# peach-xiao/EMRT

Measured on AMD Instinct MI355X. Metric: training tiles/sec at 256x256, higher is better.
Workload: dtype bf16; 1 GPU; EMRT ResNet50, Potsdam 256x256, 6 classes, batch 8 per GPU, fwd+bwd+SGD step (BASELINE configs[1]), bf16; global_batch=8, parallelism=dp1, hipgraph=True

## Files before the change

emrt_amd/csrc/bn_operand.hpp:

```cpp
#pragma once
#include "common.hpp"

namespace emrt {

#define BN_REPLICAS 8
__device__ __forceinline__ double rep_sum(const double* __restrict__ sums, int C, int idx) {
  double t = 0.0;
#pragma unroll
  for (int r = 0; r < BN_REPLICAS; ++r) t += sums[(long long)r * 2 * C + idx];
  return t;
}

struct BnChan { float mean, invstd; };
__device__ __forceinline__ BnChan bn_chan(const double* __restrict__ sums, const float* __restrict__ run_mean,
                                          const float* __restrict__ run_var, int C, int c, double inv_count, float eps) {
  BnChan o;
  if (sums) {
    const double mu = rep_sum(sums, C, c) * inv_count;
    double var = rep_sum(sums, C, C + c) * inv_count - mu * mu;
    if (var < 0.0) var = 0.0;
    o.mean = (float)mu;
    o.invstd = (float)(1.0 / sqrt(var + (double)eps));
  } else {
    o.mean = run_mean[c];
    o.invstd = rsqrtf(run_var[c] + eps);
  }
  return o;
}

__device__ __forceinline__ void bn_scale_shift(float mean, float invstd, float gamma, float beta, float& scale, float& shift) {
  scale = invstd * gamma;
  shift = fmaf(-mean, scale, beta);
}

struct BnOperand {
  const double* sums;
  double inv_count;
  float eps, momentum;
  float* mean;
  float* invstd;
  float* run_mean;
  float* run_var;
  const float* gamma;
  const float* beta;
  int relu;
};

__device__ __forceinline__ void bn_operand_preamble(const BnOperand& b, int C, float* lds, bool first) {
  for (int ch = threadIdx.x; ch < C; ch += blockDim.x) {
    const BnChan k = bn_chan(b.sums, nullptr, nullptr, C, ch, b.inv_count, b.eps);
    float sc, sh;
    bn_scale_shift(k.mean, k.invstd, b.gamma[ch], b.beta[ch], sc, sh);
    lds[ch] = sc;
    lds[C + ch] = sh;
    if (first) {
      b.mean[ch] = k.mean;
      b.invstd[ch] = k.invstd;
      if (b.run_mean) {
        const double mu = rep_sum(b.sums, C, ch) * b.inv_count;
        double var = rep_sum(b.sums, C, C + ch) * b.inv_count - mu * mu;
        if (var < 0.0) var = 0.0;
        b.run_mean[ch] = b.momentum * b.run_mean[ch] + (1.f - b.momentum) * (float)mu;
        b.run_var[ch] = b.momentum * b.run_var[ch] + (1.f - b.momentum) * (float)var;
      }
    }
  }
  __syncthreads();
}

}
```

emrt_amd/csrc/common.hpp:

```cpp
#pragma once
#include <hip/hip_runtime.h>
#include <stdint.h>
#include <stdio.h>
#include <string.h>
#include "../../include/emrt_hip.h"

#define EMRT_F32 0
#define EMRT_BF16 1
#define EMRT_F16 2

namespace emrt {

extern thread_local char g_err[512];
inline int fail(const char* fn, const char* msg) {
  snprintf(g_err, sizeof(g_err), "%s: %s", fn, msg);
  return -1;
}
inline int check_launch(const char* fn) {
  hipError_t e = hipGetLastError();
  if (e != hipSuccess) {
    snprintf(g_err, sizeof(g_err), "%s: launch failed: %s", fn, hipGetErrorString(e));
    return -2;
  }
  return 0;
}
#define EMRT_REQUIRE(cond, msg) \
  do {                          \
    if (!(cond)) return emrt::fail(__func__, msg); \
  } while (0)

struct Tuning {
  int conv_tile;
  int wgrad_split;
  int thin_cblk;
  int thin_blocks;
  int thin_ch;
  int no_thin_bwd;
  int igemm64_nst;
  int wgrad_nst;
  int pair_max;
  int msda_fwd_global;
  int msda_bwd_global;
  int msda_lds_min_pairs;
  int msda_bwd_dref_lds;
  int msda_band_halo;
  int msda_scatter_qsplit;
  int msda_scatter_cuts;
  int msda_fwd_chunks;
  int msda_fwd_threads;
  int msda_fwd_probe;
  int bn_block_kb;
  int bn_operand_blocks;
  int ln_bwd_rows;
  int ln_bwd_max_blocks;
  int ln_bwd_threads;
  int ln_atomic;
  int gn_group_blocks;
  int gn_stat_rows;
  int gn_bwd_stat_rows;
  int gn_apply_rows;
  int igemm8p_probe;
  int igemm8p_cmajor;
  int igemm8p_min_blocks;
  int wgrad8p_min_steps;
  int wgrad8p_slab;
  int wgrad8p_xcd;
  int wgrad8p_force;
  int no_ksplit128;
  int wgrad_no_overwrite;
  int no_s2_dgrad;
  int wgroup_blocks;
  int wgroup_min_steps;
  int wgroup_max;
  int wgroup8;
  int wgroup8_blocks;
  int wgroup8_min_work;
  int msda_scatter_merge;
  int msda_scatter_mfma;
  int msda_mf_bands;
  int sgd_nt;
  int mha_bwd_split;
  int mha_valu;
  int no_bna;
  int memcpy_kernel;
  int xk;
};
extern Tuning g_tune;

struct Scratch {
  void* ptr; size_t bytes; void* stream;
  unsigned* tick;
  float* xk_part;
};
constexpr size_t SCRATCH_TICK_BYTES = 65536;
constexpr int SCRATCH_TICKS = (int)(SCRATCH_TICK_BYTES / 4);
constexpr size_t SCRATCH_XK_BYTES = 8u << 20;
extern Scratch g_scratch;

struct bf16_t {
  unsigned short v;
};
struct f16_t {
  unsigned short v;
};

__device__ __forceinline__ float to_f32(float x) { return x; }
__device__ __forceinline__ float to_f32(bf16_t x) { return __uint_as_float(((uint32_t)x.v) << 16); }
__device__ __forceinline__ float to_f32(f16_t x) { return (float)__builtin_bit_cast(_Float16, x.v); }
__device__ __forceinline__ float bf16_bits_to_f32(uint32_t lo16) { return __uint_as_float(lo16 << 16); }
__device__ __forceinline__ float f16_bits_to_f32(uint32_t lo16) { return (float)__builtin_bit_cast(_Float16, (unsigned short)lo16); }

template <class T>
__device__ __forceinline__ T from_f32(float f);
template <>
__device__ __forceinline__ float from_f32<float>(float f) {
  return f;
}
template <>
__device__ __forceinline__ bf16_t from_f32<bf16_t>(float f) {
  __bf16 b = (__bf16)f;
  bf16_t r;
  r.v = __builtin_bit_cast(unsigned short, b);
  return r;
}
template <>
__device__ __forceinline__ f16_t from_f32<f16_t>(float f) {
  f16_t r;
  r.v = __builtin_bit_cast(unsigned short, (_Float16)f);
  return r;
}
typedef __attribute__((ext_vector_type(2))) _Float16 emrt_half2_t;
typedef __attribute__((ext_vector_type(2))) float emrt_float2_t;
__device__ __forceinline__ uint32_t pack_f16x2(float lo, float hi) {
  emrt_half2_t h = __builtin_convertvector((emrt_float2_t){lo, hi}, emrt_half2_t);
// ... 252 lines not shown
```

emrt_amd/csrc/elementwise.hip:

```cpp
#include "common.hpp"
#include <stdlib.h>

using namespace emrt;

thread_local char emrt::g_err[512] = {0};

extern "C" const char* emrt_last_error(void) { return emrt::g_err; }
extern "C" int emrt_abi_version(void) { return 9; }

namespace {
struct TuneEntry { const char* name; int emrt::Tuning::*field; int def; };
const TuneEntry kTune[] = {
    {"conv_tile", &emrt::Tuning::conv_tile, 0},         {"wgrad_split", &emrt::Tuning::wgrad_split, 0},
    {"thin_cblk", &emrt::Tuning::thin_cblk, 64},        {"thin_blocks", &emrt::Tuning::thin_blocks, 128},
    {"thin_ch", &emrt::Tuning::thin_ch, 8},             {"no_thin_bwd", &emrt::Tuning::no_thin_bwd, 0},
    {"pair_max", &emrt::Tuning::pair_max, 768},         {"msda_fwd_global", &emrt::Tuning::msda_fwd_global, 0},
    {"bn_block_kb", &emrt::Tuning::bn_block_kb, 8},     {"ln_atomic", &emrt::Tuning::ln_atomic, 1},
    {"msda_fwd_chunks", &emrt::Tuning::msda_fwd_chunks, 0}, {"msda_fwd_threads", &emrt::Tuning::msda_fwd_threads, 1024},
    {"msda_fwd_probe", &emrt::Tuning::msda_fwd_probe, 0}, {"wgrad_nst", &emrt::Tuning::wgrad_nst, 2},
    {"igemm64_nst", &emrt::Tuning::igemm64_nst, 3}, {"msda_bwd_global", &emrt::Tuning::msda_bwd_global, 0},
    {"msda_lds_min_pairs", &emrt::Tuning::msda_lds_min_pairs, 2048}, {"msda_bwd_dref_lds", &emrt::Tuning::msda_bwd_dref_lds, 1},
    {"gn_group_blocks", &emrt::Tuning::gn_group_blocks, 0}, {"gn_stat_rows", &emrt::Tuning::gn_stat_rows, 32},
    {"gn_bwd_stat_rows", &emrt::Tuning::gn_bwd_stat_rows, 32}, {"gn_apply_rows", &emrt::Tuning::gn_apply_rows, 8},
    {"msda_scatter_cuts", &emrt::Tuning::msda_scatter_cuts, 0}, {"msda_scatter_qsplit", &emrt::Tuning::msda_scatter_qsplit, 0}, {"msda_band_halo", &emrt::Tuning::msda_band_halo, 0},
    {"igemm8p_probe", &emrt::Tuning::igemm8p_probe, 0}, {"igemm8p_min_blocks", &emrt::Tuning::igemm8p_min_blocks, 160}, {"igemm8p_cmajor", &emrt::Tuning::igemm8p_cmajor, 0},
    {"wgrad8p_min_steps", &emrt::Tuning::wgrad8p_min_steps, 8}, {"wgrad8p_slab", &emrt::Tuning::wgrad8p_slab, 1}, {"wgrad8p_force", &emrt::Tuning::wgrad8p_force, 0}, {"wgrad8p_xcd", &emrt::Tuning::wgrad8p_xcd, 1},
    {"wgrad_no_overwrite", &emrt::Tuning::wgrad_no_overwrite, 0}, {"no_ksplit128", &emrt::Tuning::no_ksplit128, 0}, {"ln_bwd_rows", &emrt::Tuning::ln_bwd_rows, 0}, {"ln_bwd_max_blocks", &emrt::Tuning::ln_bwd_max_blocks, 0}, {"bn_operand_blocks", &emrt::Tuning::bn_operand_blocks, 0}, {"no_s2_dgrad", &emrt::Tuning::no_s2_dgrad, 0}, {"wgroup_blocks", &emrt::Tuning::wgroup_blocks, 1024}, {"wgroup_min_steps", &emrt::Tuning::wgroup_min_steps, 32}, {"wgroup_max", &emrt::Tuning::wgroup_max, 0},
    {"no_bna", &emrt::Tuning::no_bna, 0}, {"memcpy_kernel", &emrt::Tuning::memcpy_kernel, 0}, {"xk", &emrt::Tuning::xk, 0}, {"mha_valu", &emrt::Tuning::mha_valu, 0}, {"mha_bwd_split", &emrt::Tuning::mha_bwd_split, 1}, {"msda_scatter_merge", &emrt::Tuning::msda_scatter_merge, 0},
    {"wgroup8", &emrt::Tuning::wgroup8, 0}, {"wgroup8_blocks", &emrt::Tuning::wgroup8_blocks, 0}, {"wgroup8_min_work", &emrt::Tuning::wgroup8_min_work, 6000},
    {"msda_scatter_mfma", &emrt::Tuning::msda_scatter_mfma, 1}, {"sgd_nt", &emrt::Tuning::sgd_nt, 1}, {"ln_bwd_threads", &emrt::Tuning::ln_bwd_threads, 512}, {"msda_mf_bands", &emrt::Tuning::msda_mf_bands, 0},
};
emrt::Tuning tuning_from_env() {
  emrt::Tuning t;
  for (const TuneEntry& e : kTune) {
    char env[64] = "EMRT_";
    size_t n = strlen(env);
    for (const char* c = e.name; *c && n + 1 < sizeof(env); ++c) env[n++] = (char)((*c >= 'a' && *c <= 'z') ? *c - 32 : *c);
    env[n] = 0;
    const char* v = (strcmp(e.name, "msda_fwd_probe") == 0 || strcmp(e.name, "igemm8p_probe") == 0) ? nullptr : getenv(env);
    t.*(e.field) = v ? atoi(v) : e.def;
  }
  return t;
}
}
emrt::Tuning emrt::g_tune = tuning_from_env();
emrt::Scratch emrt::g_scratch = {nullptr, 0, nullptr, nullptr, nullptr};

extern "C" int emrt_set_scratch(void* ptr, size_t bytes, void* stream) {
  EMRT_REQUIRE((ptr != nullptr) == (bytes > 0) && ((uintptr_t)ptr) % 256 == 0, "scratch must be 256-byte aligned device memory (or nullptr, 0)");
  if (ptr && ptr == emrt::g_scratch.ptr && emrt::g_scratch.tick && bytes == emrt::g_scratch.bytes + emrt::SCRATCH_TICK_BYTES + emrt::SCRATCH_XK_BYTES) {
    emrt::g_scratch.stream = stream;
    return 0;
  }
  emrt::g_scratch.ptr = ptr;
  emrt::g_scratch.bytes = bytes;
  emrt::g_scratch.stream = stream;
  emrt::g_scratch.tick = nullptr;
  emrt::g_scratch.xk_part = nullptr;
  if (ptr && bytes >= (16u << 20) + emrt::SCRATCH_XK_BYTES + emrt::SCRATCH_TICK_BYTES && bytes % 256 == 0) {
    emrt::g_scratch.bytes = bytes - emrt::SCRATCH_TICK_BYTES - emrt::SCRATCH_XK_BYTES;
    emrt::g_scratch.xk_part = reinterpret_cast<float*>(static_cast<char*>(ptr) + emrt::g_scratch.bytes);
    emrt::g_scratch.tick = reinterpret_cast<unsigned*>(static_cast<char*>(ptr) + emrt::g_scratch.bytes + emrt::SCRATCH_XK_BYTES);
    if (hipMemsetAsync(emrt::g_scratch.tick, 0, emrt::SCRATCH_TICK_BYTES, (hipStream_t)stream) != hipSuccess) {
      emrt::g_scratch.tick = nullptr;
      return emrt::fail("emrt_set_scratch", "cannot zero the arrival counters");
    }
  }
  return 0;
}

extern "C" int emrt_set_tuning(const char* name, int value) {
  EMRT_REQUIRE(name, "null name");
  for (const TuneEntry& e : kTune)
    if (strcmp(e.name, name) == 0) { emrt::g_tune.*(e.field) = value; return 0; }
  return emrt::fail("emrt_set_tuning", "unknown knob");
}
extern "C" int emrt_get_tuning(const char* name, int* value) {
  EMRT_REQUIRE(name && value, "null pointer");
  for (const TuneEntry& e : kTune)
    if (strcmp(e.name, name) == 0) { *value = emrt::g_tune.*(e.field); return 0; }
  return emrt::fail("emrt_get_tuning", "unknown knob");
}

static inline int ew_grid(long long total) {
  long long g = (total + 255) / 256;
  if (g > 8192) g = 8192;
  if (g < 1) g = 1;
  return (int)g;
}

template <class T>
__global__ __launch_bounds__(256) void add_kernel(const T* __restrict__ a, const T* __restrict__ b, T* __restrict__ out, long long n4,
                                                  long long period4) {
  for (long long i = (long long)blockIdx.x * blockDim.x + threadIdx.x; i < n4; i += (long long)gridDim.x * blockDim.x) {
    float x[4], y[4];
    Vec4<T>::load(a + i * 4, x);
    Vec4<T>::load(b + ((n4 | period4) <= 0xffffffffll ? (long long)((unsigned)i % (unsigned)period4) : i % period4) * 4, y);
#pragma unroll
    for (int e = 0; e < 4; ++e) x[e] += y[e];
    Vec4<T>::store(out + i * 4, x);
// ... 381 lines not shown
```

emrt_amd/csrc/norm.hip:

```cpp
#include "common.hpp"
#include "bn_operand.hpp"
#include <stdlib.h>

using namespace emrt;

template <class T, int MODE>
__global__ __launch_bounds__(256) void col_reduce_kernel(const T* __restrict__ x, int ldx, const T* __restrict__ dy, int lddy,
                                                         const T* __restrict__ y, int ldy, const float* __restrict__ mean,
                                                         const float* __restrict__ invstd, long long M, int C, int tx_n,
                                                         float* __restrict__ partial, long long rpb, long long bs,
                                                         double* __restrict__ dsums, float* __restrict__ facc,
                                                         const float* __restrict__ mgamma = nullptr, const float* __restrict__ mbeta = nullptr) {
  __shared__ float red[256 * 8];
  const int ty_n = 256 / tx_n;
  const int tx = threadIdx.x % tx_n, ty = threadIdx.x / tx_n;
  const int c = (blockIdx.y * tx_n + tx) * 4;
  float s0[4] = {0, 0, 0, 0}, s1[4] = {0, 0, 0, 0};
  if (c < C) {
    float mu[4] = {0, 0, 0, 0}, is[4] = {1, 1, 1, 1};
    float msc[MODE == 3 ? 4 : 1], msh[MODE == 3 ? 4 : 1];
    if (MODE == 1 || MODE == 3) {
#pragma unroll
      for (int e = 0; e < 4; ++e) { mu[e] = mean[c + e]; is[e] = invstd[c + e]; }
      if constexpr (MODE == 3) {
// ... 44 lines not shown
  if (ty == 0 && c < C) {
    for (int t = 1; t < ty_n; ++t) {
#pragma unroll
      for (int e = 0; e < 4; ++e) { s0[e] += red[(t * tx_n + tx) * 8 + e]; s1[e] += red[(t * tx_n + tx) * 8 + 4 + e]; }
    }
    if (dsums) {
      double* rep = dsums + (long long)(blockIdx.x & 7) * 2 * C;
#pragma unroll
      for (int e = 0; e < 4; ++e) { atomicAdd(rep + c + e, (double)s0[e]); atomicAdd(rep + C + c + e, (double)s1[e]); }
    } else if (facc) {
#pragma unroll
      for (int e = 0; e < 4; ++e)
        if (c + e < C) atomicAdd(facc + c + e, s0[e]);
    } else {
      float* pp = partial + (long long)blockIdx.x * 2 * C;
#pragma unroll
      for (int e = 0; e < 4; ++e) { pp[c + e] = s0[e]; pp[C + c + e] = s1[e]; }
    }
  }
}

static inline void col_reduce_geometry(long long M, int C, int& tx_n, int& gx, int& gy) {
  int quads = (C + 3) / 4;
  tx_n = 64;
  while (tx_n > 1 && tx_n / 2 >= quads) tx_n /= 2;
  gy = (quads + tx_n - 1) / tx_n;
  int ty_n = 256 / tx_n;
  long long want = (M + (long long)ty_n * 8 - 1) / ((long long)ty_n * 8);
  long long cap = 512 / gy;
  if (cap < 1) cap = 1;
  gx = (int)(want < 1 ? 1 : (want > cap ? cap : want));
}

__global__ __launch_bounds__(256) void bn_sum_partials_kernel(const float* __restrict__ partial, int nblk, int C, float* __restrict__ sums ) {
  __shared__ double red[8][33];
  const int cx = threadIdx.x & 31, py = threadIdx.x >> 5;
  const int c = blockIdx.x * 32 + cx;
  double s = 0.0;
  if (c < 2 * C)
    for (int b = py; b < nblk; b += 8) s += (double)partial[(long long)b * 2 * C + c];
  red[py][cx] = s;
  __syncthreads();
  if (py == 0 && c < 2 * C) {
    double t = 0.0;
#pragma unroll
    for (int k = 0; k < 8; ++k) t += red[k][cx];
    sums[c] = (float)t;
  }
}

__global__ __launch_bounds__(256) void partials_acc_kernel(const float* __restrict__ partial, int nblk, int C, float* __restrict__ dgamma,
                                                          float* __restrict__ dbeta) {
  __shared__ double red[8][33];
  const int cx = threadIdx.x & 31, py = threadIdx.x >> 5;
  const int c = blockIdx.x * 32 + cx;
  double s = 0.0;
  if (c < 2 * C)
    for (int b = py; b < nblk; b += 8) s += (double)partial[(long long)b * 2 * C + c];
  red[py][cx] = s;
  __syncthreads();
  if (py == 0 && c < 2 * C) {
    double t = 0.0;
#pragma unroll
    for (int k = 0; k < 8; ++k) t += red[k][cx];
    if (c < C) { if (dbeta) dbeta[c] += (float)t; }
    else if (dgamma) dgamma[c - C] += (float)t;
  }
}

__global__ void bn_bwd_finalize_kernel(const float* __restrict__ sums, int C, float* __restrict__ dgamma, float* __restrict__ dbeta) {
  const int c = blockIdx.x * blockDim.x + threadIdx.x;
  if (c >= C) return;
  if (dbeta) dbeta[c] += sums[c];
  if (dgamma) dgamma[c] += sums[C + c];
}

template <class T, bool JOIN = false>
__global__ __launch_bounds__(512) void bn_apply_kernel(const T* __restrict__ x, int ldx, const T* __restrict__ res, int ldres,
                                                       T* __restrict__ y, int ldy, const double* __restrict__ sums, double inv_count,
                                                       float eps, float momentum, float* __restrict__ mean_out,
                                                       float* __restrict__ invstd_out, float* __restrict__ run_mean,
                                                       float* __restrict__ run_var, const float* __restrict__ gamma,
                                                       const float* __restrict__ beta, long long M, int C, int relu, int rows_per_pass,
                                                       BnOperand rbn) {
  const int quads = C / 4;
  const int c = (threadIdx.x % quads) * 4;
  const int lane_row = threadIdx.x / quads;
  const long long rstep = (long long)gridDim.x * rows_per_pass;
  long long r = (long long)blockIdx.x * rows_per_pass + lane_row;
  float v[4], w[4];
  if (r < M) {
    Vec4<T>::load(x + r * ldx + c, v);
    if (res) Vec4<T>::load(res + r * ldres + c, w);
  }
  extern __shared__ float bn_lds[];
  if constexpr (JOIN) bn_operand_preamble(rbn, C, bn_lds + 2 * C, blockIdx.x == 0);
  for (int ch = threadIdx.x; ch < C; ch += blockDim.x) {
    const BnChan k = bn_chan(sums, run_mean, run_var, C, ch, inv_count, eps);
    float scale, shift;
    bn_scale_shift(k.mean, k.invstd, gamma[ch], beta[ch], scale, shift);
    bn_lds[ch] = scale;
    bn_lds[C + ch] = shift;
    if (sums && blockIdx.x == 0) {
      mean_out[ch] = k.mean;
      invstd_out[ch] = k.invstd;
      if (run_mean) {
        const double mu = rep_sum(sums, C, ch) * inv_count;
        double var = rep_sum(sums, C, C + ch) * inv_count - mu * mu;
        if (var < 0.0) var = 0.0;
        run_mean[ch] = momentum * run_mean[ch] + (1.f - momentum) * (float)mu;
        run_var[ch] = momentum * run_var[ch] + (1.f - momentum) * (float)var;
      }
    }
  }
  __syncthreads();
  float sc[4], sh[4], rsc[JOIN ? 4 : 1], rsh[JOIN ? 4 : 1];
#pragma unroll
  for (int e = 0; e < 4; ++e) {
    sc[e] = bn_lds[c + e]; sh[e] = bn_lds[C + c + e];
    if constexpr (JOIN) { rsc[e] = bn_lds[2 * C + c + e]; rsh[e] = bn_lds[3 * C + c + e]; }
  }
  while (r < M) {
    const long long rn = r + rstep;
    float vn[4], wn[4], o[4];
    if (rn < M) {
      Vec4<T>::load(x + rn * ldx + c, vn);
      if (res) Vec4<T>::load(res + rn * ldres + c, wn);
    }
#pragma unroll
    for (int e = 0; e < 4; ++e) o[e] = fmaf(v[e], sc[e], sh[e]);
    if (res) {
      if constexpr (JOIN) {
#pragma unroll
        for (int e = 0; e < 4; ++e) o[e] += to_f32(from_f32<T>(fmaf(w[e], rsc[e], rsh[e])));
      } else {
#pragma unroll
        for (int e = 0; e < 4; ++e) o[e] += w[e];
      }
    }
    if (relu) {
#pragma unroll
      for (int e = 0; e < 4; ++e) o[e] = fmaxf(o[e], 0.f);
    }
    Vec4<T>::store(y + r * ldy + c, o);
#pragma unroll
    for (int e = 0; e < 4; ++e) { v[e] = vn[e]; w[e] = wn[e]; }
    r = rn;
  }
}

template <class T, bool MX = false>
__global__ __launch_bounds__(512) void bn_bwd_dx_kernel(const T* __restrict__ x, int ldx, const T* __restrict__ dy, int lddy,
                                                        const T* __restrict__ y, int ldy, T* __restrict__ dx, int lddx,
                                                        T* __restrict__ dres, int lddres, const float* __restrict__ mean,
                                                        const float* __restrict__ invstd, const float* __restrict__ gamma,
                                                        const double* __restrict__ sums, const double* __restrict__ lsums,
                                                        double inv_count, float* __restrict__ dgamma, float* __restrict__ dbeta,
                                                        long long M, int C, int rows_per_pass, const float* __restrict__ beta_y, int sums_vs_x,
                                                        const float* __restrict__ mbeta) {
  const int quads = C / 4;
  const int c = (threadIdx.x % quads) * 4;
  const int lane_row = threadIdx.x / quads;
  const long long rstep = (long long)gridDim.x * rows_per_pass;
  long long r = (long long)blockIdx.x * rows_per_pass + lane_row;
  float v[4], g[4], yy[4];
  if (r < M) {
    Vec4<T>::load(x + r * ldx + c, v);
    Vec4<T>::load(dy + r * lddy + c, g);
    if (y) Vec4<T>::load(y + r * ldy + c, yy);
  }
  extern __shared__ float bn_lds[];
  for (int ch = threadIdx.x; ch < C; ch += blockDim.x) {
    const double t0 = rep_sum(sums, C, ch);
    double t1 = rep_sum(sums, C, C + ch);
    if (beta_y) {
      const double gm = (double)gamma[ch];
      t1 = gm != 0.0 ? (t1 - (double)beta_y[ch] * t0) / gm : 0.0;
    }
    if (sums_vs_x) t1 = (t1 - (double)mean[ch] * t0) * (double)invstd[ch];
    bn_lds[ch] = (float)(t0 * inv_count);
    bn_lds[C + ch] = (float)(t1 * inv_count);
    if (blockIdx.x == 0) {
      if (dbeta) dbeta[ch] += (float)(lsums ? rep_sum(lsums, C, ch) : t0);
      if (dgamma) dgamma[ch] += (float)(lsums ? rep_sum(lsums, C, C + ch) : t1);
    }
  }
  __syncthreads();
  float mu[4], is[4], k0[4], k1[4], gi[4], msc[MX ? 4 : 1], msh[MX ? 4 : 1];
#pragma unroll
  for (int e = 0; e < 4; ++e) {
    mu[e] = mean[c + e];
    is[e] = invstd[c + e];
    gi[e] = gamma[c + e] * is[e];
    k0[e] = bn_lds[c + e];
    k1[e] = bn_lds[C + c + e];
    if constexpr (MX) bn_scale_shift(mu[e], is[e], gamma[c + e], mbeta[c + e], msc[e], msh[e]);
  }
  while (r < M) {
    const long long rn = r + rstep;
    float vn[4], gn[4], yn[4], o[4];
    if (rn < M) {
      Vec4<T>::load(x + rn * ldx + c, vn);
      Vec4<T>::load(dy + rn * lddy + c, gn);
      if (y) Vec4<T>::load(y + rn * ldy + c, yn);
    }
    if (y) {
#pragma unroll
      for (int e = 0; e < 4; ++e) g[e] = yy[e] > 0.f ? g[e] : 0.f;
    }
    if constexpr (MX) {
#pragma unroll
      for (int e = 0; e < 4; ++e) g[e] = fmaf(v[e], msc[e], msh[e]) > 0.f ? g[e] : 0.f;
    }
#pragma unroll
    for (int e = 0; e < 4; ++e) o[e] = gi[e] * (g[e] - k0[e] - (v[e] - mu[e]) * is[e] * k1[e]);
    Vec4<T>::store(dx + r * lddx + c, o);
    if (dres) Vec4<T>::store(dres + r * lddres + c, g);
#pragma unroll
    for (int e = 0; e < 4; ++e) { v[e] = vn[e]; g[e] = gn[e]; yy[e] = yn[e]; }
    r = rn;
  }
}


__device__ __forceinline__ float gelu_f(float x) { return 0.5f * x * (1.f + erff(x * 0.70710678118654752f)); }
__device__ __forceinline__ float gelu_grad_f(float x) {
  return 0.5f * (1.f + erff(x * 0.70710678118654752f)) + x * 0.3989422804014327f * __expf(-0.5f * x * x);
}

template <class T>
__global__ __launch_bounds__(256) void gn_stats_kernel(const T* __restrict__ x, int ldx, long long x_bs, double* __restrict__ sums,
                                                       int HW, int C, int G, int pix_per_block) {
  __shared__ float red[256 * 2];
  const int quads = C / 4, lanes = 256 / quads;
  const int q = threadIdx.x % quads, ty = threadIdx.x / quads;
  const int n = blockIdx.y, c = q * 4, cpg = C / G;
  const int p0 = blockIdx.x * pix_per_block;
  int p1 = p0 + pix_per_block;
  if (p1 > HW) p1 = HW;
  const T* xp = x + (long long)n * x_bs;
  float s0 = 0.f, s1 = 0.f;
  for (int p = p0 + ty; p < p1; p += lanes) {
    float v[4];
    Vec4<T>::load(xp + (long long)p * ldx + c, v);
#pragma unroll
    for (int e = 0; e < 4; ++e) { s0 += v[e]; s1 = fmaf(v[e], v[e], s1); }
  }
  red[threadIdx.x * 2] = s0;
  red[threadIdx.x * 2 + 1] = s1;
  __syncthreads();
  if ((int)threadIdx.x < G) {
    const int g = threadIdx.x;
    double a = 0.0, b = 0.0;
    const int q0 = g * cpg / 4, q1 = (g + 1) * cpg / 4;
    for (int t = 0; t < lanes; ++t)
      for (int qq = q0; qq < q1; ++qq) { a += red[(t * quads + qq) * 2]; b += red[(t * quads + qq) * 2 + 1]; }
    atomicAdd(sums + ((long long)n * G + g) * 2, a);
    atomicAdd(sums + ((long long)n * G + g) * 2 + 1, b);
  }
}

template <class T>
__global__ __launch_bounds__(256) void gn_apply_kernel(const T* __restrict__ x, int ldx, long long x_bs, const T* __restrict__ res,
                                                       int ldres, long long res_bs, T* __restrict__ out, int ldout, long long out_bs,
                                                       const float* __restrict__ gamma, const float* __restrict__ beta,
                                                       const double* __restrict__ sums, float* __restrict__ mean_out,
                                                       float* __restrict__ rstd_out, int HW, int C, int G, float eps, int gelu,
                                                       int pix_per_block) {
  const int quads = C / 4, lanes = 256 / quads;
  const int q = threadIdx.x % quads, ty = threadIdx.x / quads;
  const int n = blockIdx.y, c = q * 4, cpg = C / G, g = c / cpg;
  const double cnt = (double)HW * cpg;
  const double mu_d = sums[((long long)n * G + g) * 2] / cnt;
  double var = sums[((long long)n * G + g) * 2 + 1] / cnt - mu_d * mu_d;
  if (var < 0.0) var = 0.0;
  const float mu = (float)mu_d, rs = (float)(1.0 / sqrt(var + (double)eps));
  if (mean_out && blockIdx.x == 0 && ty == 0 && (c % cpg) == 0) { mean_out[n * G + g] = mu; rstd_out[n * G + g] = rs; }
  float sc[4], sh[4];
// ... 711 lines not shown
        }
        float gm[4];
#pragma unroll
        for (int e = 0; e < 4; ++e) gm[e] = gamma[c + e];
#pragma unroll
        for (int k = 0; k < R; ++k) {
          const float wk = ok[k] ? 1.f : 0.f;
#pragma unroll
          for (int e = 0; e < 4; ++e) {
            xh[k][j][e] = (zz[k][e] - mu[k]) * rs[k];
            gd[k][j][e] = gm[e] * dd[k][e];
            s0[k] += gd[k][j][e];
            s1[k] = fmaf(gd[k][j][e], xh[k][j][e], s1[k]);
            dg[j][e] = fmaf(wk * dd[k][e], xh[k][j][e], dg[j][e]);
            db[j][e] = fmaf(wk, dd[k][e], db[j][e]);
          }
        }
      }
    }
#pragma unroll
    for (int k = 0; k < R; ++k) { s0[k] = wave_sum(s0[k]) / (float)C; s1[k] = wave_sum(s1[k]) / (float)C; }
#pragma unroll
    for (int j = 0; j < NQ; ++j) {
      const int c = j * 256 + lane * 4;
      if (j < nq && c < C) {
#pragma unroll
        for (int k = 0; k < R; ++k) {
          if (!ok[k]) continue;
          float o[4];
#pragma unroll
          for (int e = 0; e < 4; ++e) o[e] = rs[k] * (gd[k][j][e] - s0[k] - xh[k][j][e] * s1[k]);
          if (addend) {
            float ad[4], oa[4];
            Vec4<T>::load(addend + row[k] * C + c, ad);
#pragma unroll
            for (int e = 0; e < 4; ++e) oa[e] = o[e] + ad[e];
            Vec4<T>::store(dz + row[k] * C + c, oa);
          } else {
            Vec4<T>::store(dz + row[k] * C + c, o);
          }
          if (dzb) {
            if (pdrop > 0.f) {
              uint32_t hq[2];
              drop_quad(sd, salt, (unsigned long long)(row[k] * C + c) >> 2, hq);
              const uint32_t thr = drop_thr16(pdrop);
#pragma unroll
              for (int e = 0; e < 4; ++e)
                o[e] = drop_quad_keep(hq, e, thr) ? to_f32(from_f32<T>(o[e])) * ks : 0.f;
            }
            Vec4<T>::store(dzb + row[k] * C + c, o);
          }
        }
      }
    }
  }
#pragma unroll
  for (int j = 0; j < NQ; ++j) {
    const int c = j * 256 + lane * 4;
    if (j < nq && c < C) {
#pragma unroll
      for (int e = 0; e < 4; ++e) { sm[(wv * 2 + 0) * C + c + e] = db[j][e]; sm[(wv * 2 + 1) * C + c + e] = dg[j][e]; }
    }
  }
  __syncthreads();
  for (int c = threadIdx.x; c < C; c += TPB) {
    float b0 = 0.f, g0 = 0.f;
    for (int w = 0; w < NWV; ++w) { b0 += sm[(w * 2 + 0) * C + c]; g0 += sm[(w * 2 + 1) * C + c]; }
    if (dgamma_direct || dbeta_direct) {
      if (dbeta_direct) atomicAdd(dbeta_direct + c, b0);
      if (dgamma_direct) atomicAdd(dgamma_direct + c, g0);
    } else {
      partial[(long long)blockIdx.x * 2 * C + c] = b0;
      partial[(long long)blockIdx.x * 2 * C + C + c] = g0;
    }
  }
}

extern "C" size_t emrt_colreduce_workspace_bytes(long long M, int C) {
  int tx, gx, gy;
  col_reduce_geometry(M, C, tx, gx, gy);
  return ((size_t)gx * 2 * C + 2 * (size_t)C) * sizeof(float);
}

static inline bool bn_rowgeom(long long M, int C, int& threads, int& rows_per_pass, int& grid) {
  const int quads = C / 4;
  if (quads <= 256) { if (256 % quads) return false; threads = 256; rows_per_pass = 256 / quads; }
  else if (quads <= 512) { threads = quads; rows_per_pass = 1; }
  else return false;
  const long long per_block = (long long)(g_tune.bn_block_kb > 0 ? g_tune.bn_block_kb : 8) * 1024;
  long long g = (M * C * 2 + per_block - 1) / per_block;
  const long long gmax = (M + rows_per_pass - 1) / rows_per_pass;
  if (g < 64) g = 64;
  if (g > 4096) g = 4096;
  if (g > gmax) g = gmax;
  if (g < 1) g = 1;
  grid = (int)g;
  return true;
}

extern "C" int emrt_bn_stats(const void* x, int ldx, long long M, int C, double* sums, int dtype, void* stream) {
  EMRT_REQUIRE_TRAIN_DTYPE(dtype);
  EMRT_REQUIRE(x && sums, "null pointer");
  EMRT_REQUIRE(C % 4 == 0 && ldx % 4 == 0, "C and ld must be multiples of 4");
  int tx, gx, gy;
  col_reduce_geometry(M, C, tx, gx, gy);
  hipStream_t st = (hipStream_t)stream;
  return with_train_dtype("emrt_bn_stats", dtype, [&](auto t) {
    using T = decltype(t);
    hipLaunchKernelGGL((col_reduce_kernel<T, 0>), dim3(gx, gy), dim3(256), 0, st, (const T*)x, ldx, nullptr, 0, nullptr, 0, nullptr, nullptr, M, C, tx, nullptr, M, 0LL, sums, nullptr);
    return check_launch("emrt_bn_stats");
  });
}

extern "C" int emrt_bn_apply(const void* x, int ldx, const void* res, int ldres, void* y, int ldy, const double* sums, double count,
                             float eps, float momentum, float* mean, float* invstd, float* run_mean, float* run_var,
                             const float* gamma, const float* beta, long long M, int C, int relu, int dtype, void* stream) {
  EMRT_REQUIRE_FWD_DTYPE(dtype);
  EMRT_REQUIRE(x && y && gamma && beta, "null pointer");
  EMRT_REQUIRE(sums ? (mean && invstd) : (run_mean && run_var), "training needs mean/invstd outputs, eval needs running statistics");
  EMRT_REQUIRE(C % 4 == 0 && ldx % 4 == 0 && ldy % 4 == 0 && (!res || ldres % 4 == 0), "C and ld must be multiples of 4");
  int threads, rpp, grid;
  EMRT_REQUIRE(bn_rowgeom(M, C, threads, rpp, grid), "unsupported channel count (C/4 must divide 256, or C <= 2048)");
  hipStream_t st = (hipStream_t)stream;
  const double inv_count = sums ? 1.0 / count : 0.0;
  BnOperand none;
  memset(&none, 0, sizeof(none));
  return with_fwd_dtype("emrt_bn_apply", dtype, [&](auto t) {
    using T = decltype(t);
    hipLaunchKernelGGL((bn_apply_kernel<T>), dim3(grid), dim3(threads), (size_t)2 * C * sizeof(float), st, (const T*)x, ldx, (const T*)res, ldres, (T*)y, ldy, sums, inv_count, eps, momentum, mean, invstd, run_mean, run_var, gamma, beta, M, C, relu, rpp, none);
    return check_launch("emrt_bn_apply");
  });
}

extern "C" int emrt_bn_apply_join(const void* x, int ldx, const void* res_raw, int ldres, void* y, int ldy, const double* sums, double count,
                                  float eps, float momentum, float* mean, float* invstd, float* run_mean, float* run_var, const float* gamma,
                                  const float* beta, const double* r_sums, double r_count, float r_eps, float r_momentum, float* r_mean,
                                  float* r_invstd, float* r_run_mean, float* r_run_var, const float* r_gamma, const float* r_beta, long long M,
                                  int C, int relu, int dtype, void* stream) {
  EMRT_REQUIRE_TRAIN_DTYPE(dtype);
  EMRT_REQUIRE(x && res_raw && y && gamma && beta && sums && mean && invstd, "null pointer");
  EMRT_REQUIRE(r_sums && r_mean && r_invstd && r_gamma && r_beta && r_count > 0.0 && count > 0.0 && (r_run_mean != nullptr) == (r_run_var != nullptr),
               "the shortcut's BatchNorm needs sums, mean, invstd, gamma, beta and a positive count");
  EMRT_REQUIRE(C % 4 == 0 && ldx % 4 == 0 && ldy % 4 == 0 && ldres % 4 == 0, "C and ld must be multiples of 4");
  int threads, rpp, grid;
  EMRT_REQUIRE(bn_rowgeom(M, C, threads, rpp, grid), "unsupported channel count (C/4 must divide 256, or C <= 2048)");
  BnOperand r;
  r.sums = r_sums; r.inv_count = 1.0 / r_count; r.eps = r_eps; r.momentum = r_momentum; r.mean = r_mean; r.invstd = r_invstd;
  r.run_mean = r_run_mean; r.run_var = r_run_var; r.gamma = r_gamma; r.beta = r_beta; r.relu = 0;
  hipStream_t st = (hipStream_t)stream;
  const double inv_count = 1.0 / count;
  const size_t lds = (size_t)4 * C * sizeof(float);
  return with_train_dtype("emrt_bn_apply_join", dtype, [&](auto t) {
    using T = decltype(t);
    hipLaunchKernelGGL((bn_apply_kernel<T, true>), dim3(grid), dim3(threads), lds, st, (const T*)x, ldx, (const T*)res_raw, ldres, (T*)y, ldy, sums, inv_count, eps, momentum, mean, invstd, run_mean, run_var, gamma, beta, M, C, relu, rpp, r);
    return check_launch("emrt_bn_apply_join");
  });
}

__global__ __launch_bounds__(256) void bn_fold_kernel(const float* __restrict__ params, const float* __restrict__ buffers,
                                                      const long long* __restrict__ desc, float eps, float* __restrict__ out) {
  const long long* d = desc + 7 * (long long)blockIdx.x;
  const float* gamma = params + d[0];
  const float* beta = params + d[1];
  const float* mean = buffers + d[2];
  const float* var = buffers + d[3];
  const int C = (int)d[4];
  float* o = out + d[5];
  const float* cbias = d[6] >= 0 ? params + d[6] : nullptr;
  for (int c = threadIdx.x; c < C; c += blockDim.x) {
    const float sc = gamma[c] * rsqrtf(var[c] + eps);
    o[c] = sc;
    o[C + c] = beta[c] + ((cbias ? cbias[c] : 0.f) - mean[c]) * sc;
  }
}
extern "C" int emrt_bn_fold(const float* params, const float* buffers, const long long* desc, int n, float eps, float* out, void* stream) {
  EMRT_REQUIRE(params && buffers && desc && out && n > 0, "null pointer");
  hipLaunchKernelGGL(bn_fold_kernel, dim3(n), dim3(256), 0, (hipStream_t)stream, params, buffers, desc, eps, out);
  return check_launch("emrt_bn_fold");
}

extern "C" int emrt_bn_bwd_reduce(const void* x, int ldx, const void* dy, int lddy, const void* y, int ldy, const float* mean,
                                  const float* invstd, long long M, int C, double* sums, const float* mask_gamma, const float* mask_beta,
                                  int dtype, void* stream) {
  EMRT_REQUIRE_TRAIN_DTYPE(dtype);
  EMRT_REQUIRE(x && dy && mean && invstd && sums, "null pointer");
  EMRT_REQUIRE((mask_gamma != nullptr) == (mask_beta != nullptr) && !(mask_beta && y), "mask_gamma and mask_beta come together and replace y");
  EMRT_REQUIRE(C % 4 == 0 && ldx % 4 == 0 && lddy % 4 == 0 && (!y || ldy % 4 == 0), "C and ld must be multiples of 4");
  int tx, gx, gy;
  col_reduce_geometry(M, C, tx, gx, gy);
  hipStream_t st = (hipStream_t)stream;
  return with_train_dtype("emrt_bn_bwd_reduce", dtype, [&](auto t) {
    using T = decltype(t);
    if (mask_beta) {
      hipLaunchKernelGGL((col_reduce_kernel<T, 3>), dim3(gx, gy), dim3(256), 0, st, (const T*)x, ldx, (const T*)dy, lddy, (const T*)nullptr, 0, mean, invstd, M, C, tx, nullptr, M, 0LL, sums, nullptr, mask_gamma, mask_beta);
      return check_launch("emrt_bn_bwd_reduce");
    }
    hipLaunchKernelGGL((col_reduce_kernel<T, 1>), dim3(gx, gy), dim3(256), 0, st, (const T*)x, ldx, (const T*)dy, lddy, (const T*)y, ldy, mean, invstd, M, C, tx, nullptr, M, 0LL, sums, nullptr);
    return check_launch("emrt_bn_bwd_reduce");
  });
}

extern "C" int emrt_bn_bwd_dx(const void* x, int ldx, const void* dy, int lddy, const void* y, int ldy, void* dx, int lddx,
                              void* dres, int lddres, const float* mean, const float* invstd, const float* gamma,
                              const double* sums, const double* local_sums, double count, float* dgamma, float* dbeta, long long M,
                              int C, const float* beta_y_moments, int sums_vs_x, const float* mask_beta, int dtype, void* stream) {
  EMRT_REQUIRE_TRAIN_DTYPE(dtype);
  EMRT_REQUIRE(x && dy && dx && mean && invstd && gamma && sums, "null pointer");
  EMRT_REQUIRE(!(mask_beta && (y || beta_y_moments || sums_vs_x)), "mask_beta (ReLU mask re-derived from x) excludes y and the fused-sum forms");
  EMRT_REQUIRE(C % 4 == 0 && ldx % 4 == 0 && lddy % 4 == 0 && lddx % 4 == 0, "C and ld must be multiples of 4");
  int threads, rpp, grid;
  EMRT_REQUIRE(bn_rowgeom(M, C, threads, rpp, grid), "unsupported channel count (C/4 must divide 256, or C <= 2048)");
  hipStream_t st = (hipStream_t)stream;
  return with_train_dtype("emrt_bn_bwd_dx", dtype, [&](auto t) {
    using T = decltype(t);
    if (mask_beta) {
      hipLaunchKernelGGL((bn_bwd_dx_kernel<T, true>), dim3(grid), dim3(threads), (size_t)2 * C * sizeof(float), st, (const T*)x, ldx, (const T*)dy, lddy, (const T*)nullptr, 0, (T*)dx, lddx, (T*)dres, lddres, mean, invstd, gamma, sums, local_sums, 1.0 / count, dgamma, dbeta, M, C, rpp, nullptr, 0, mask_beta);
      return check_launch("emrt_bn_bwd_dx");
    }
    hipLaunchKernelGGL((bn_bwd_dx_kernel<T>), dim3(grid), dim3(threads), (size_t)2 * C * sizeof(float), st, (const T*)x, ldx, (const T*)dy, lddy, (const T*)y, ldy, (T*)dx, lddx, (T*)dres, lddres, mean, invstd, gamma, sums, local_sums, 1.0 / count, dgamma, dbeta, M, C, rpp, beta_y_moments, sums_vs_x, mask_beta);
    return check_launch("emrt_bn_bwd_dx");
  });
}

template <class T>
__global__ __launch_bounds__(256) void colsum_scalar_kernel(const T* __restrict__ x, int ldx, long long rpb, long long bs, long long M,
                                                            float* __restrict__ dbias) {
  __shared__ float red[4];
  const int c = blockIdx.x;
  float s = 0.f;
  for (long long r = threadIdx.x; r < M; r += 256) {
    const long long bb = r / rpb;
    s += to_f32(x[bb * bs + (r - bb * rpb) * ldx + c]);
  }
  s = wave_sum(s);
  if ((threadIdx.x & 63) == 0) red[threadIdx.x >> 6] = s;
  __syncthreads();
  if (threadIdx.x == 0) dbias[c] += red[0] + red[1] + red[2] + red[3];
}

extern "C" int emrt_colsum_acc(const void* x, int ldx, long long rows_per_batch, long long x_bs, long long M, int C, float* dbias,
                               void* workspace, int dtype, void* stream) {
  EMRT_REQUIRE_TRAIN_DTYPE(dtype);
  EMRT_REQUIRE(rows_per_batch > 0, "bad batch geometry");
  EMRT_REQUIRE(x && dbias && workspace, "null pointer");
  return with_train_dtype("emrt_colsum_acc", dtype, [&](auto t) {
    using T = decltype(t);
    if (C % 4 != 0 || ldx % 4 != 0 || x_bs % 4 != 0) {
      hipStream_t st0 = (hipStream_t)stream;
      hipLaunchKernelGGL((colsum_scalar_kernel<T>), dim3(C), dim3(256), 0, st0, (const T*)x, ldx, rows_per_batch, x_bs, M, dbias);
      return check_launch("emrt_colsum_acc(scalar)");
    }
    int tx, gx, gy;
    col_reduce_geometry(M, C, tx, gx, gy);
    hipStream_t st = (hipStream_t)stream;
    float* partial = (float*)workspace;
    const bool direct = g_tune.ln_atomic != 0;
    hipLaunchKernelGGL((col_reduce_kernel<T, 2>), dim3(gx, gy), dim3(256), 0, st, (const T*)x, ldx, nullptr, 0, nullptr, 0, nullptr, nullptr, M, C, tx, partial, rows_per_batch, x_bs, nullptr, direct ? dbias : nullptr);
    if (!direct) hipLaunchKernelGGL(partials_acc_kernel, dim3((C + 31) / 32), dim3(256), 0, st, partial, gx, C, (float*)nullptr, dbias);
    return check_launch("emrt_colsum_acc");
  });
}

struct ColsumLevelsArgs {
  const void* x[8];
  int T, L, B, Lv, C;
  int start[4], count[4];
  float* dst;
};
template <class T>
__global__ __launch_bounds__(256) void colsum_levels_kernel(ColsumLevelsArgs a) {
  const int quads = a.C / 4;
  const int cq = threadIdx.x % quads, lane_row = threadIdx.x / quads, lanes = 256 / quads;
  const int l = blockIdx.y;
  float acc[4] = {0.f, 0.f, 0.f, 0.f};
  const int npair = a.T * a.B;
  for (int r = blockIdx.x * lanes + lane_row; r < a.count[l]; r += gridDim.x * lanes) {
    const long long row = a.start[l] + r;
    for (int p0 = blockIdx.z; p0 < npair; p0 += 4 * gridDim.z) {
      float v[4][4];
#pragma unroll
      for (int u = 0; u < 4; ++u) {
        const int pp = p0 + u * gridDim.z;
        const int t = pp < npair ? pp / a.B : 0, b = pp < npair ? pp - t * a.B : 0;
        Vec4<T>::load((const T*)a.x[t] + ((long long)b * a.Lv + row) * a.C + cq * 4, v[u]);
        if (pp >= npair) { v[u][0] = 0.f; v[u][1] = 0.f; v[u][2] = 0.f; v[u][3] = 0.f; }
      }
#pragma unroll
      for (int u = 0; u < 4; ++u)
#pragma unroll
        for (int e = 0; e < 4; ++e) acc[e] += v[u][e];
    }
  }
  __shared__ float red[256 * 4];
#pragma unroll
  for (int e = 0; e < 4; ++e) red[(lane_row * quads + cq) * 4 + e] = acc[e];
  __syncthreads();
  for (int c = threadIdx.x; c < a.C; c += 256) {
    float s = 0.f;
    for (int q = 0; q < lanes; ++q) s += red[(q * quads + c / 4) * 4 + (c & 3)];
    atomicAdd(a.dst + (long long)l * a.C + c, s);
  }
}
// ... 430 lines not shown
```

Before: 1005 tiles/s.

## Slice BatchNorm apply and backward kernels over channel blocks with 2D grid

BN apply, apply-join and backward-dx kernels now split channels into slices of 64 across grid.x, with row blocks on grid.y. Each block computes scale/shift only for its slice, so the per-block preamble (double-precision replica sums) and LDS footprint shrink for wide layers. The per-block byte budget also becomes automatic, scaling with tensor size between 2KB and 8KB instead of a fixed 8KB. Rows per pass grow for wide channels, and per-slice row blocks are divided by the slice count, which changes occupancy and memory access width per row.

```diff
diff --git a/emrt_amd/csrc/bn_operand.hpp b/emrt_amd/csrc/bn_operand.hpp
--- a/emrt_amd/csrc/bn_operand.hpp
+++ b/emrt_amd/csrc/bn_operand.hpp
@@ -46,13 +46,15 @@
   int relu;
 };
 
-__device__ __forceinline__ void bn_operand_preamble(const BnOperand& b, int C, float* lds, bool first) {
-  for (int ch = threadIdx.x; ch < C; ch += blockDim.x) {
+__device__ __forceinline__ void bn_operand_preamble(const BnOperand& b, int C, float* lds, bool first, int c0 = 0, int cs = -1) {
+  if (cs < 0) cs = C;
+  for (int l = threadIdx.x; l < cs; l += blockDim.x) {
+    const int ch = c0 + l;
     const BnChan k = bn_chan(b.sums, nullptr, nullptr, C, ch, b.inv_count, b.eps);
     float sc, sh;
     bn_scale_shift(k.mean, k.invstd, b.gamma[ch], b.beta[ch], sc, sh);
-    lds[ch] = sc;
-    lds[C + ch] = sh;
+    lds[l] = sc;
+    lds[cs + l] = sh;
     if (first) {
       b.mean[ch] = k.mean;
       b.invstd[ch] = k.invstd;
diff --git a/emrt_amd/csrc/common.hpp b/emrt_amd/csrc/common.hpp
--- a/emrt_amd/csrc/common.hpp
+++ b/emrt_amd/csrc/common.hpp
@@ -50,6 +50,7 @@
   int msda_fwd_threads;
   int msda_fwd_probe;
   int bn_block_kb;
+  int bn_slice_c;
   int bn_operand_blocks;
   int ln_bwd_rows;
   int ln_bwd_max_blocks;
diff --git a/emrt_amd/csrc/elementwise.hip b/emrt_amd/csrc/elementwise.hip
--- a/emrt_amd/csrc/elementwise.hip
+++ b/emrt_amd/csrc/elementwise.hip
@@ -15,7 +15,8 @@
     {"thin_cblk", &emrt::Tuning::thin_cblk, 64},        {"thin_blocks", &emrt::Tuning::thin_blocks, 128},
     {"thin_ch", &emrt::Tuning::thin_ch, 8},             {"no_thin_bwd", &emrt::Tuning::no_thin_bwd, 0},
     {"pair_max", &emrt::Tuning::pair_max, 768},         {"msda_fwd_global", &emrt::Tuning::msda_fwd_global, 0},
-    {"bn_block_kb", &emrt::Tuning::bn_block_kb, 8},     {"ln_atomic", &emrt::Tuning::ln_atomic, 1},
+    {"bn_block_kb", &emrt::Tuning::bn_block_kb, 0},     {"ln_atomic", &emrt::Tuning::ln_atomic, 1},
+    {"bn_slice_c", &emrt::Tuning::bn_slice_c, 0},
     {"msda_fwd_chunks", &emrt::Tuning::msda_fwd_chunks, 0}, {"msda_fwd_threads", &emrt::Tuning::msda_fwd_threads, 1024},
     {"msda_fwd_probe", &emrt::Tuning::msda_fwd_probe, 0}, {"wgrad_nst", &emrt::Tuning::wgrad_nst, 2},
     {"igemm64_nst", &emrt::Tuning::igemm64_nst, 3}, {"msda_bwd_global", &emrt::Tuning::msda_bwd_global, 0},
diff --git a/emrt_amd/csrc/norm.hip b/emrt_amd/csrc/norm.hip
--- a/emrt_amd/csrc/norm.hip
+++ b/emrt_amd/csrc/norm.hip
@@ -150,26 +150,30 @@
                                                        float* __restrict__ invstd_out, float* __restrict__ run_mean,
                                                        float* __restrict__ run_var, const float* __restrict__ gamma,
                                                        const float* __restrict__ beta, long long M, int C, int relu, int rows_per_pass,
-                                                       BnOperand rbn) {
-  const int quads = C / 4;
-  const int c = (threadIdx.x % quads) * 4;
+                                                       int cs, BnOperand rbn) {
+  const int quads = cs / 4;
+  const int c0 = blockIdx.x * cs;
+  const int lc = (threadIdx.x % quads) * 4;
+  const int c = c0 + lc;
   const int lane_row = threadIdx.x / quads;
-  const long long rstep = (long long)gridDim.x * rows_per_pass;
-  long long r = (long long)blockIdx.x * rows_per_pass + lane_row;
+  const bool first = blockIdx.y == 0;
+  const long long rstep = (long long)gridDim.y * rows_per_pass;
+  long long r = (long long)blockIdx.y * rows_per_pass + lane_row;
   float v[4], w[4];
   if (r < M) {
     Vec4<T>::load(x + r * ldx + c, v);
     if (res) Vec4<T>::load(res + r * ldres + c, w);
   }
   extern __shared__ float bn_lds[];
-  if constexpr (JOIN) bn_operand_preamble(rbn, C, bn_lds + 2 * C, blockIdx.x == 0);
-  for (int ch = threadIdx.x; ch < C; ch += blockDim.x) {
+  if constexpr (JOIN) bn_operand_preamble(rbn, C, bn_lds + 2 * cs, first, c0, cs);
+  for (int l = threadIdx.x; l < cs; l += blockDim.x) {
+    const int ch = c0 + l;
     const BnChan k = bn_chan(sums, run_mean, run_var, C, ch, inv_count, eps);
     float scale, shift;
     bn_scale_shift(k.mean, k.invstd, gamma[ch], beta[ch], scale, shift);
-    bn_lds[ch] = scale;
-    bn_lds[C + ch] = shift;
-    if (sums && blockIdx.x == 0) {
+    bn_lds[l] = scale;
+    bn_lds[cs + l] = shift;
+    if (sums && first) {
       mean_out[ch] = k.mean;
       invstd_out[ch] = k.invstd;
       if (run_mean) {
@@ -185,8 +189,8 @@
   float sc[4], sh[4], rsc[JOIN ? 4 : 1], rsh[JOIN ? 4 : 1];
 #pragma unroll
   for (int e = 0; e < 4; ++e) {
-    sc[e] = bn_lds[c + e]; sh[e] = bn_lds[C + c + e];
-    if constexpr (JOIN) { rsc[e] = bn_lds[2 * C + c + e]; rsh[e] = bn_lds[3 * C + c + e]; }
+    sc[e] = bn_lds[lc + e]; sh[e] = bn_lds[cs + lc + e];
+    if constexpr (JOIN) { rsc[e] = bn_lds[2 * cs + lc + e]; rsh[e] = bn_lds[3 * cs + lc + e]; }
   }
   while (r < M) {
     const long long rn = r + rstep;
@@ -224,13 +228,15 @@
                                                         const float* __restrict__ invstd, const float* __restrict__ gamma,
                                                         const double* __restrict__ sums, const double* __restrict__ lsums,
                                                         double inv_count, float* __restrict__ dgamma, float* __restrict__ dbeta,
-                                                        long long M, int C, int rows_per_pass, const float* __restrict__ beta_y, int sums_vs_x,
+                                                        long long M, int C, int rows_per_pass, int cs, const float* __restrict__ beta_y, int sums_vs_x,
                                                         const float* __restrict__ mbeta) {
-  const int quads = C / 4;
-  const int c = (threadIdx.x % quads) * 4;
+  const int quads = cs / 4;
+  const int c0 = blockIdx.x * cs;
+  const int lc = (threadIdx.x % quads) * 4;
+  const int c = c0 + lc;
   const int lane_row = threadIdx.x / quads;
-  const long long rstep = (long long)gridDim.x * rows_per_pass;
-  long long r = (long long)blockIdx.x * rows_per_pass + lane_row;
+  const long long rstep = (long long)gridDim.y * rows_per_pass;
+  long long r = (long long)blockIdx.y * rows_per_pass + lane_row;
   float v[4], g[4], yy[4];
   if (r < M) {
     Vec4<T>::load(x + r * ldx + c, v);
@@ -238,7 +244,8 @@
     if (y) Vec4<T>::load(y + r * ldy + c, yy);
   }
   extern __shared__ float bn_lds[];
-  for (int ch = threadIdx.x; ch < C; ch += blockDim.x) {
+  for (int l = threadIdx.x; l < cs; l += blockDim.x) {
+    const int ch = c0 + l;
     const double t0 = rep_sum(sums, C, ch);
     double t1 = rep_sum(sums, C, C + ch);
     if (beta_y) {
@@ -246,9 +253,9 @@
       t1 = gm != 0.0 ? (t1 - (double)beta_y[ch] * t0) / gm : 0.0;
     }
     if (sums_vs_x) t1 = (t1 - (double)mean[ch] * t0) * (double)invstd[ch];
-    bn_lds[ch] = (float)(t0 * inv_count);
-    bn_lds[C + ch] = (float)(t1 * inv_count);
-    if (blockIdx.x == 0) {
+    bn_lds[l] = (float)(t0 * inv_count);
+    bn_lds[cs + l] = (float)(t1 * inv_count);
+    if (blockIdx.y == 0) {
       if (dbeta) dbeta[ch] += (float)(lsums ? rep_sum(lsums, C, ch) : t0);
       if (dgamma) dgamma[ch] += (float)(lsums ? rep_sum(lsums, C, C + ch) : t1);
     }
@@ -260,8 +267,8 @@
     mu[e] = mean[c + e];
     is[e] = invstd[c + e];
     gi[e] = gamma[c + e] * is[e];
-    k0[e] = bn_lds[c + e];
-    k1[e] = bn_lds[C + c + e];
+    k0[e] = bn_lds[lc + e];
+    k1[e] = bn_lds[cs + lc + e];
     if constexpr (MX) bn_scale_shift(mu[e], is[e], gamma[c + e], mbeta[c + e], msc[e], msh[e]);
   }
   while (r < M) {
@@ -1139,19 +1146,33 @@
   return ((size_t)gx * 2 * C + 2 * (size_t)C) * sizeof(float);
 }
 
-static inline bool bn_rowgeom(long long M, int C, int& threads, int& rows_per_pass, int& grid) {
+static inline int bn_slice_auto(long long M, int C) {
+  (void)M; (void)C;
+  return 64;
+}
+static inline long long bn_block_bytes_auto(long long M, int C) {
+  const long long b = M * C * 2 / 1024;
+  return b < 2048 ? 2048 : b > 8192 ? 8192 : b;
+}
+
+static inline bool bn_rowgeom(long long M, int C, int& threads, int& rows_per_pass, int& cs, dim3& grid) {
   const int quads = C / 4;
   if (quads <= 256) { if (256 % quads) return false; threads = 256; rows_per_pass = 256 / quads; }
   else if (quads <= 512) { threads = quads; rows_per_pass = 1; }
   else return false;
-  const long long per_block = (long long)(g_tune.bn_block_kb > 0 ? g_tune.bn_block_kb : 8) * 1024;
+  cs = g_tune.bn_slice_c > 0 ? g_tune.bn_slice_c : bn_slice_auto(M, C);
+  if (cs < 64 || cs >= C || cs % 4 || C % cs || 256 % (cs / 4)) cs = C;
+  if (cs < C) { threads = 256; rows_per_pass = 256 / (cs / 4); }
+  const int slices = C / cs;
+  const long long per_block = g_tune.bn_block_kb > 0 ? (long long)g_tune.bn_block_kb * 1024 : bn_block_bytes_auto(M, C);
   long long g = (M * C * 2 + per_block - 1) / per_block;
   const long long gmax = (M + rows_per_pass - 1) / rows_per_pass;
   if (g < 64) g = 64;
   if (g > 4096) g = 4096;
+  g = (g + slices - 1) / slices;
   if (g > gmax) g = gmax;
   if (g < 1) g = 1;
-  grid = (int)g;
+  grid = dim3(slices, (unsigned)g);
   return true;
 }
 
@@ -1176,15 +1197,16 @@
   EMRT_REQUIRE(x && y && gamma && beta, "null pointer");
   EMRT_REQUIRE(sums ? (mean && invstd) : (run_mean && run_var), "training needs mean/invstd outputs, eval needs running statistics");
   EMRT_REQUIRE(C % 4 == 0 && ldx % 4 == 0 && ldy % 4 == 0 && (!res || ldres % 4 == 0), "C and ld must be multiples of 4");
-  int threads, rpp, grid;
-  EMRT_REQUIRE(bn_rowgeom(M, C, threads, rpp, grid), "unsupported channel count (C/4 must divide 256, or C <= 2048)");
+  int threads, rpp, cs;
+  dim3 grid;
+  EMRT_REQUIRE(bn_rowgeom(M, C, threads, rpp, cs, grid), "unsupported channel count (C/4 must divide 256, or C <= 2048)");
   hipStream_t st = (hipStream_t)stream;
   const double inv_count = sums ? 1.0 / count : 0.0;
   BnOperand none;
   memset(&none, 0, sizeof(none));
   return with_fwd_dtype("emrt_bn_apply", dtype, [&](auto t) {
     using T = decltype(t);
-    hipLaunchKernelGGL((bn_apply_kernel<T>), dim3(grid), dim3(threads), (size_t)2 * C * sizeof(float), st, (const T*)x, ldx, (const T*)res, ldres, (T*)y, ldy, sums, inv_count, eps, momentum, mean, invstd, run_mean, run_var, gamma, beta, M, C, relu, rpp, none);
+    hipLaunchKernelGGL((bn_apply_kernel<T>), grid, dim3(threads), (size_t)2 * cs * sizeof(float), st, (const T*)x, ldx, (const T*)res, ldres, (T*)y, ldy, sums, inv_count, eps, momentum, mean, invstd, run_mean, run_var, gamma, beta, M, C, relu, rpp, cs, none);
     return check_launch("emrt_bn_apply");
   });
 }
@@ -1199,17 +1221,18 @@
   EMRT_REQUIRE(r_sums && r_mean && r_invstd && r_gamma && r_beta && r_count > 0.0 && count > 0.0 && (r_run_mean != nullptr) == (r_run_var != nullptr),
                "the shortcut's BatchNorm needs sums, mean, invstd, gamma, beta and a positive count");
   EMRT_REQUIRE(C % 4 == 0 && ldx % 4 == 0 && ldy % 4 == 0 && ldres % 4 == 0, "C and ld must be multiples of 4");
-  int threads, rpp, grid;
-  EMRT_REQUIRE(bn_rowgeom(M, C, threads, rpp, grid), "unsupported channel count (C/4 must divide 256, or C <= 2048)");
+  int threads, rpp, cs;
+  dim3 grid;
+  EMRT_REQUIRE(bn_rowgeom(M, C, threads, rpp, cs, grid), "unsupported channel count (C/4 must divide 256, or C <= 2048)");
   BnOperand r;
   r.sums = r_sums; r.inv_count = 1.0 / r_count; r.eps = r_eps; r.momentum = r_momentum; r.mean = r_mean; r.invstd = r_invstd;
   r.run_mean = r_run_mean; r.run_var = r_run_var; r.gamma = r_gamma; r.beta = r_beta; r.relu = 0;
   hipStream_t st = (hipStream_t)stream;
   const double inv_count = 1.0 / count;
-  const size_t lds = (size_t)4 * C * sizeof(float);
+  const size_t lds = (size_t)4 * cs * sizeof(float);
   return with_train_dtype("emrt_bn_apply_join", dtype, [&](auto t) {
     using T = decltype(t);
-    hipLaunchKernelGGL((bn_apply_kernel<T, true>), dim3(grid), dim3(threads), lds, st, (const T*)x, ldx, (const T*)res_raw, ldres, (T*)y, ldy, sums, inv_count, eps, momentum, mean, invstd, run_mean, run_var, gamma, beta, M, C, relu, rpp, r);
+    hipLaunchKernelGGL((bn_apply_kernel<T, true>), grid, dim3(threads), lds, st, (const T*)x, ldx, (const T*)res_raw, ldres, (T*)y, ldy, sums, inv_count, eps, momentum, mean, invstd, run_mean, run_var, gamma, beta, M, C, relu, rpp, cs, r);
     return check_launch("emrt_bn_apply_join");
   });
 }
@@ -1265,16 +1288,17 @@
   EMRT_REQUIRE(x && dy && dx && mean && invstd && gamma && sums, "null pointer");
   EMRT_REQUIRE(!(mask_beta && (y || beta_y_moments || sums_vs_x)), "mask_beta (ReLU mask re-derived from x) excludes y and the fused-sum forms");
   EMRT_REQUIRE(C % 4 == 0 && ldx % 4 == 0 && lddy % 4 == 0 && lddx % 4 == 0, "C and ld must be multiples of 4");
-  int threads, rpp, grid;
-  EMRT_REQUIRE(bn_rowgeom(M, C, threads, rpp, grid), "unsupported channel count (C/4 must divide 256, or C <= 2048)");
+  int threads, rpp, cs;
+  dim3 grid;
+  EMRT_REQUIRE(bn_rowgeom(M, C, threads, rpp, cs, grid), "unsupported channel count (C/4 must divide 256, or C <= 2048)");
   hipStream_t st = (hipStream_t)stream;
   return with_train_dtype("emrt_bn_bwd_dx", dtype, [&](auto t) {
     using T = decltype(t);
     if (mask_beta) {
-      hipLaunchKernelGGL((bn_bwd_dx_kernel<T, true>), dim3(grid), dim3(threads), (size_t)2 * C * sizeof(float), st, (const T*)x, ldx, (const T*)dy, lddy, (const T*)nullptr, 0, (T*)dx, lddx, (T*)dres, lddres, mean, invstd, gamma, sums, local_sums, 1.0 / count, dgamma, dbeta, M, C, rpp, nullptr, 0, mask_beta);
+      hipLaunchKernelGGL((bn_bwd_dx_kernel<T, true>), grid, dim3(threads), (size_t)2 * cs * sizeof(float), st, (const T*)x, ldx, (const T*)dy, lddy, (const T*)nullptr, 0, (T*)dx, lddx, (T*)dres, lddres, mean, invstd, gamma, sums, local_sums, 1.0 / count, dgamma, dbeta, M, C, rpp, cs, nullptr, 0, mask_beta);
       return check_launch("emrt_bn_bwd_dx");
     }
-    hipLaunchKernelGGL((bn_bwd_dx_kernel<T>), dim3(grid), dim3(threads), (size_t)2 * C * sizeof(float), st, (const T*)x, ldx, (const T*)dy, lddy, (const T*)y, ldy, (T*)dx, lddx, (T*)dres, lddres, mean, invstd, gamma, sums, local_sums, 1.0 / count, dgamma, dbeta, M, C, rpp, beta_y_moments, sums_vs_x, mask_beta);
+    hipLaunchKernelGGL((bn_bwd_dx_kernel<T>), grid, dim3(threads), (size_t)2 * cs * sizeof(float), st, (const T*)x, ldx, (const T*)dy, lddy, (const T*)y, ldy, (T*)dx, lddx, (T*)dres, lddres, mean, invstd, gamma, sums, local_sums, 1.0 / count, dgamma, dbeta, M, C, rpp, cs, beta_y_moments, sums_vs_x, mask_beta);
     return check_launch("emrt_bn_bwd_dx");
   });
 }
```

New measurement: 1045 tiles/s (median of 6 runs). 4.0% higher.
